# leonzheng2/Safe-Exploration-with-Simulator-in-RL-algorithms

Hardware: AMD Instinct MI355X
Metric: env-steps/sec (higher is better)
Workload: dtype f64; 1 GPU; ARS V2 iteration, 3-segment swimmer, 512 directions/GPU x 2 rollouts x H=1000 (BASELINE configs[2] per GPU); directions_total=512, directions_per_gpu=512, horizon=1000, segments=3, trajectory_capture=True, full_covariance=True, parallelism=directions sharded over 1 GPU(s), 1 all-gather/iteration, ranks_seen=1

## Files before the change

include/swimmer_hip.h:

```cpp
#ifndef SWIMMER_HIP_H
#define SWIMMER_HIP_H

#include <stdint.h>

#ifdef __cplusplus
extern "C" {
#endif

#define SW_ABI_VERSION 3
#define SW_MAX_SEGMENTS 8

#define SW_OK 0
#define SW_ERR_NULL 1
#define SW_ERR_SEGMENTS 2
#define SW_ERR_SIZE 3
#define SW_ERR_PARAM 4
#define SW_ERR_LAUNCH 5

#define SW_STATUS_OK 0
#define SW_STATUS_SINGULAR 1
#define SW_STATUS_NONFINITE 2
#define SW_STATUS_RANGE 4

#define SW_FLAG_ROLLOUT_LANE 1
// ... 110 lines not shown
int sw_ars_iteration_rollouts_f64(sw_ars_pipeline *pl, int slot, const sw_params *p,
                                  int64_t n_dir_total, int64_t dir_begin, int64_t n_dir,
                                  int32_t H, const double *deltas_host ,
                                  double *deltas_dev, const double *policy, double nu,
                                  const double *mean, const double *inv_std, double *returns,
                                  double *traj, double *moments, double *cov_acc,
                                  int32_t *status, void *stream);

int sw_ars_iteration_update_f64(sw_ars_pipeline *pl, int slot, const sw_params *p,
                                int64_t n_dir, const double *gathered, int32_t world,
                                int64_t chunk, int64_t rows_chunk, const double *deltas_dev,
                                double *policy, double alpha, double b, int64_t top_b,
                                double *running, int64_t n_new_states, double *mean,
                                double *inv_std, double *sigma_out, void *stream);

#ifdef __cplusplus
}
#endif
#endif
```

safe-exploration-with-simulator-in-rl-algorithms_amd/_lib.py:

```python
import ctypes
import os

import numpy as np
import torch

from . import _build

ABI_VERSION = 3
MAX_SEGMENTS = 8

ERR_NAMES = {0: "SW_OK", 1: "SW_ERR_NULL", 2: "SW_ERR_SEGMENTS", 3: "SW_ERR_SIZE",
             4: "SW_ERR_PARAM", 5: "SW_ERR_LAUNCH"}
STATUS_SINGULAR = 1
STATUS_NONFINITE = 2
STATUS_RANGE = 4
FLAG_ROLLOUT_LANE = 1
FLAG_ROLLOUT_QUAD = 2
FLAG_MODEL_TWIN = 4
COST_ABS_OBS = 0
COST_MAX_ABS_THETADOT = 1


class SwParams(ctypes.Structure):
    _fields_ = [("n", ctypes.c_int32), ("flags", ctypes.c_int32), ("l_i", ctypes.c_double),
# ... 88 lines not shown
                                                     ctypes.c_void_p, ctypes.c_int64,
                                                     ctypes.c_int64, ctypes.c_int64,
                                                     ctypes.c_int32, ctypes.c_void_p,
                                                     ctypes.c_void_p, ctypes.c_void_p,
                                                     ctypes.c_double] + [ctypes.c_void_p] * 8),
    "sw_ars_iteration_update_f64": (ctypes.c_int, [ctypes.c_void_p, ctypes.c_int,
                                                   ctypes.c_void_p, ctypes.c_int64,
                                                   ctypes.c_void_p, ctypes.c_int32,
                                                   ctypes.c_int64, ctypes.c_int64,
                                                   ctypes.c_void_p, ctypes.c_void_p,
                                                   ctypes.c_double, ctypes.c_double,
                                                   ctypes.c_int64, ctypes.c_void_p,
                                                   ctypes.c_int64, ctypes.c_void_p,
                                                   ctypes.c_void_p, ctypes.c_void_p,
                                                   ctypes.c_void_p]),
    "sw_ars_update_gathered_f64": (ctypes.c_int, [ctypes.c_void_p, ctypes.c_int64,
                                                  ctypes.c_void_p, ctypes.c_int32,
                                                  ctypes.c_int64, ctypes.c_int64,
                                                  ctypes.c_void_p, ctypes.c_void_p,
                                                  ctypes.c_double, ctypes.c_double,
                                                  ctypes.c_int64, ctypes.c_void_p,
                                                  ctypes.c_int64, ctypes.c_void_p,
                                                  ctypes.c_void_p, ctypes.c_void_p,
                                                  ctypes.c_void_p]),
}
EXPORTED_SYMBOLS = tuple(_PROTOTYPES)


def library_path():
    return _build.LIB_PATH
# ... 73 lines not shown
```

safe-exploration-with-simulator-in-rl-algorithms_amd/ars/ars_agent.py:

```python
import os

import numpy as np
import torch
import torch.distributed as dist

from .. import kernels
from .._lib import (SwParams, SwimmerHipError, kernel_flags, numpy_global_uniform_pm1,
                    require_gpu)
from .database import Database
from .environment import Environment
from . import sharding as _sh
from .sharding import (all_gather_segments, returns_from_segments, segment_len,
                       shard_bounds)


class ARSAgent(object):

    def __init__(self, real_env_param, agent_param, data_path=None, seed=None,
                 guess_param=None, approx_error=None, sim_thresh=None, *, device=None,
                 process_group=None, record_trajectories=False, full_covariance=True,
                 top_b=0, rollout_kernel="auto", direct_rccl=None):
        if agent_param.safe:
            raise NotImplementedError(
                "safe exploration (ars_agent.py:144-157) gates every real rollout on a "
# ... 177 lines not shown
                           self.agent_param.b, 0, sigma_out=self._sigma)

    def run_iteration_async(self, deltas=None, want_returns=True):
        ap = self.agent_param
        i = self._pipe.next_slot()
        self._it += 1
        self._pipe.host_slot_wait(i)
        if self.record_trajectories:
            self._policy_snapshot = self._policy.cpu().numpy()
        host = self._deltas_host_np[i]
        if deltas is None:
            numpy_global_uniform_pm1(host)
        else:
            host[...] = deltas
        self._deltas, self._traj = self._deltas2[i], self._traj2[i]
        self._pipe.rollouts(i, self.params, ap.N, self.lo, self.n_local, ap.H,
                            self._deltas_host[i], self._deltas, self._policy, ap.nu,
                            self._mean, self._inv_std, self._returns_local, self._traj,
                            self._moments_local,
                            self._cov_acc if self._traj is not None else None, self._status)
        if self._coll_events is not None and (self.world > 1 or _sh._FORCE_COLLECTIVE):
            e0 = torch.cuda.Event(enable_timing=True)
            e1 = torch.cuda.Event(enable_timing=True)
            e0.record()
            gathered = self._exchange()
            e1.record()
            self._coll_events.append((e0, e1))
        else:
            gathered = self._exchange()
        n_new = 2 * ap.N * ap.H
        self._pipe.update(i, self.params, ap.N, gathered, self.world, self.chunk,
                          self.rows_chunk, self._deltas, self._policy, ap.alpha, ap.b,
                          self.top_b, self._running, n_new, self._mean, self._inv_std,
                          self._sigma)
        if self.v2:
            self.n_saved_states += n_new
        if self.record_trajectories and self._traj is not None:
            self.database.add_device_batch(self._traj.clone(),
                                           self._rollout_policies(host.copy()))
        if not want_returns:
            return None
        return returns_from_segments(gathered, ap.N, self.world, self.chunk)

    def _rollout_policies(self, deltas):
        P = self._policy_snapshot
        out = np.empty((2 * self.n_local, self.m, self.d))
        nd = self.agent_param.nu * np.asarray(deltas)[self.lo:self.hi]
        out[0::2] = P + nd
        out[1::2] = P - nd
# ... 95 lines not shown
```

safe-exploration-with-simulator-in-rl-algorithms_amd/csrc/swimmer_kernels.hip:

```cpp
#include <hip/hip_runtime.h>
#include <math.h>
#include <stdint.h>
#include <climits>
#include <cstdlib>
#include <cstring>
#include <new>
#include <type_traits>
#include <utility>
#include <vector>

#include <chrono>
#include "../../include/swimmer_hip.h"
#include "swimmer_device.h"
#include "swimmer_quad3.h"
#include "swimmer_oct3.h"
#include "swimmer_row.h"
#include "swimmer_twin.h"

#define SW_PIN_LOOP(PAD) asm volatile(".p2align 6\n\t.fill %0, 4, 0xbf800000" ::"n"(PAD))
#ifndef SW_OCT_UNROLL
#define SW_OCT_UNROLL 8
#endif
#ifdef SW_OCT_LOOP_PAD
constexpr int oct_loop_pad(bool, bool) { return SW_OCT_LOOP_PAD; }
// ... 1840 lines not shown
}

constexpr int kTopBMaxDirs = 6144;

__device__ __forceinline__ bool rank_used_global(const GatherView &g, int32_t n_dir, int64_t top_b, int32_t i)
{
    const double ki = fmax(ret_at(g, i, 0), ret_at(g, i, 1));
    int64_t rank = 0;
    for (int32_t j = 0; j < n_dir; ++j) {
        const double kj = fmax(ret_at(g, j, 0), ret_at(g, j, 1));
        rank += (kj > ki) || (kj == ki && j > i);
    }
    return rank < top_b;
}

constexpr int kUpdMaxDirs = kTopBMaxDirs;
constexpr int kTopBSortDirs = 2048;

template <int BLOCK>
__global__ void __launch_bounds__(BLOCK)
ars_update_kernel(int d, int md, int32_t n_dir, GatherView gv,
                  const double *__restrict__ deltas, double *__restrict__ policy, double alpha,
                  double b, int64_t top_b, double *__restrict__ running, double n_new,
                  double *__restrict__ mean, double *__restrict__ inv_std,
                  double *__restrict__ sigma_out)
{
    __shared__ double sh2[BLOCK / kWave][2];
    __shared__ double rp_s[kUpdMaxDirs], rm_s[kUpdMaxDirs];
    __shared__ unsigned char flag[kUpdMaxDirs];
    const int e = blockIdx.x;
// ... 4 lines not shown
        double dcol[kMaxPer];
        if (in_lds) {
#pragma unroll
            for (int q = 0; q < kMaxPer; ++q) {
                const int32_t i = threadIdx.x + q * BLOCK;
                dcol[q] = (i < n_dir) ? deltas[(int64_t)i * md + e] : 0.0;
            }
            for (int32_t i = threadIdx.x; i < n_dir; i += BLOCK) {
                rp_s[i] = ret_at(gv, i, 0);
                rm_s[i] = ret_at(gv, i, 1);
            }
            __syncthreads();
            if (select && n_dir <= kTopBSortDirs) {
                __shared__ double skey[kTopBSortDirs];
                __shared__ uint16_t sidx[kTopBSortDirs];
                uint32_t P2 = 2;
                while (P2 < (uint32_t)n_dir) P2 <<= 1;
                for (uint32_t i = threadIdx.x; i < P2; i += BLOCK) {
                    double k = -HUGE_VAL;
                    if (i < (uint32_t)n_dir) {
                        const double a = rp_s[i], b = rm_s[i];
                        k = (b > a) ? b : a;
                        k = (k != k) ? HUGE_VAL : k;
                    }
                    skey[i] = k;
                    sidx[i] = (uint16_t)i;
                }
                __syncthreads();
                for (uint32_t k = 2; k <= P2; k <<= 1) {
                    for (uint32_t j = k >> 1; j > 0; j >>= 1) {
                        for (uint32_t t = threadIdx.x; t < P2 / 2; t += BLOCK) {
                            const uint32_t lo = ((t & ~(j - 1u)) << 1) | (t & (j - 1u)), hi = lo | j;
                            const double ka = skey[lo], kb = skey[hi];
                            const uint32_t ia = sidx[lo], ib = sidx[hi];
                            const bool a_first = (ia < (uint32_t)n_dir) &&
                                                 ((ib >= (uint32_t)n_dir) || ka > kb || (ka == kb && ia > ib));
                            const bool best_first = (lo & k) == 0;
                            if (a_first != best_first) {
                                skey[lo] = kb;
                                skey[hi] = ka;
                                sidx[lo] = (uint16_t)ib;
                                sidx[hi] = (uint16_t)ia;
                            }
                        }
                        __syncthreads();
                    }
                }
                for (uint32_t pos = threadIdx.x; pos < P2; pos += BLOCK) {
                    const uint32_t i = sidx[pos];
                    if (i < (uint32_t)n_dir) flag[i] = (int64_t)pos < top_b;
                }
                __syncthreads();
            } else if (select) {
                for (int32_t i = threadIdx.x; i < n_dir; i += BLOCK) {
                    const double ki = fmax(rp_s[i], rm_s[i]);
                    int32_t rank = 0;
                    for (int32_t j = 0; j < n_dir; ++j) {
                        const double kj = fmax(rp_s[j], rm_s[j]);
                        rank += (kj > ki) || (kj == ki && j > i);
                    }
                    flag[i] = rank < top_b;
                }
                __syncthreads();
            }
        }
        auto rplus = [&](int32_t i) { return in_lds ? rp_s[i] : ret_at(gv, i, 0); };
        auto rminus = [&](int32_t i) { return in_lds ? rm_s[i] : ret_at(gv, i, 1); };
// ... 2 lines not shown
            return in_lds ? (flag[i] != 0) : rank_used_global(gv, n_dir, top_b, i);
        };
        double s = 0.0, cnt = 0.0;
        for (int32_t i = threadIdx.x; i < n_dir; i += BLOCK)
            if (dir_used(i)) {
                s += rplus(i) + rminus(i);
                cnt += 2.0;
            }
        block_sum2<BLOCK>(s, cnt, sh2);
        const double mu = s / cnt;
        double v = 0.0, g = 0.0;
        if (in_lds) {
#pragma unroll
            for (int q = 0; q < kMaxPer; ++q) {
                const int32_t i = threadIdx.x + q * BLOCK;
                if (i < n_dir && dir_used(i)) {
                    const double rp = rp_s[i], rm = rm_s[i];
                    const double a = rp - mu, c = rm - mu;
                    v += a * a + c * c;
                    g = __builtin_fma(rp - rm, dcol[q], g);
                }
            }
        } else {
            for (int32_t i = threadIdx.x; i < n_dir; i += BLOCK)
                if (dir_used(i)) {
                    const double rp = rplus(i), rm = rminus(i);
                    const double a = rp - mu, c = rm - mu;
                    v += a * a + c * c;
                    g = __builtin_fma(rp - rm, deltas[(int64_t)i * md + e], g);
                }
        }
        block_sum2<BLOCK>(v, g, sh2);
        if (threadIdx.x == 0) {
            const double sigma = sqrt(v / cnt);
            const double div = (top_b > 0) ? 0.5 * cnt : b;
            const double grad = g / (div * sigma);
            policy[e] = policy[e] + alpha * grad;
            if (e == 0 && sigma_out) *sigma_out = sigma;
        }
    } else if (running != nullptr) {
        constexpr int kMaxCols = 2 * (2 * SW_MAX_SEGMENTS + 2);
        constexpr int kMaxGroups = BLOCK / 12;
        __shared__ double part[kMaxGroups][kMaxCols];
        __shared__ double bsum[kMaxCols];
        const int cols = 2 * d, G = BLOCK / cols;
        const int rg = threadIdx.x / cols, j = threadIdx.x - rg * cols;
        const int32_t total = gv.world * gv.rows_chunk;
        if (rg < G) {
            double acc = 0.0;
            for (int32_t g0 = rg; g0 < total; g0 += 8 * G) {
                double v[8];
#pragma unroll
                for (int q = 0; q < 8; ++q) {
                    const int32_t g = g0 + q * G;
// ... 4 lines not shown
                    }
                }
#pragma unroll
                for (int q = 0; q < 8; ++q) acc += v[q];
            }
            part[rg][j] = acc;
        }
        __syncthreads();
        if (threadIdx.x < cols) {
            double t = part[0][threadIdx.x];
            for (int g = 1; g < G; ++g) t += part[g][threadIdx.x];
            bsum[threadIdx.x] = t;
        }
        __syncthreads();
        const double n0 = running[0], n1 = n0 + n_new;
        if (threadIdx.x < d && n_new > 0.0) {
            const int c_ = threadIdx.x;
            const double s1 = bsum[c_], s2 = bsum[d + c_];
            const double mb = s1 / n_new;
            const double m2b = __builtin_fma(-s1, mb, s2);
            const double mr = running[1 + c_], m2 = running[1 + d + c_];
            const double delta = mb - mr;
            const double mr1 = __builtin_fma(delta, n_new / n1, mr);
            const double m21 = (m2 + m2b) + delta * delta * (n0 * (n_new / n1));
            running[1 + c_] = mr1;
            running[1 + d + c_] = m21;
            const double c = (c_ >= 2 && (c_ & 1) == 0) ? kHalfPi : 0.0;
            mean[c_] = c + mr1;
            inv_std[c_] = 1.0 / sqrt(m21 / (n1 - 1.0));
        }
        __syncthreads();
        if (threadIdx.x == 0) running[0] = n1;
    }
}

__global__ void __launch_bounds__(256) issue_probe_kernel(int32_t trips, int32_t mode, double *out)
{
    double a0 = 1.0 + threadIdx.x, a1 = a0 + 1, a2 = a0 + 2, a3 = a0 + 3, a4 = a0 + 4, a5 = a0 + 5,
           a6 = a0 + 6, a7 = a0 + 7;
    const double m = 1.0000001, c = 1e-9;
    int b0 = threadIdx.x, b1 = b0 + 1, b2 = b0 + 2, b3 = b0 + 3, b4 = b0 + 4, b5 = b0 + 5, b6 = b0 + 6,
        b7 = b0 + 7;
#define SW_FMA8 "v_fma_f64 %0, %0, %8, %9\n v_fma_f64 %1, %1, %8, %9\n v_fma_f64 %2, %2, %8, %9\n" \
                "v_fma_f64 %3, %3, %8, %9\n v_fma_f64 %4, %4, %8, %9\n v_fma_f64 %5, %5, %8, %9\n" \
                "v_fma_f64 %6, %6, %8, %9\n v_fma_f64 %7, %7, %8, %9\n"
#define SW_MOV8 "v_mov_b32 %0, %1\n v_mov_b32 %1, %2\n v_mov_b32 %2, %3\n v_mov_b32 %3, %4\n" \
                "v_mov_b32 %4, %5\n v_mov_b32 %5, %6\n v_mov_b32 %6, %7\n v_mov_b32 %7, %0\n"
    if (mode == 0) {
        for (int32_t t = 0; t < trips; ++t)
// ... 374 lines not shown
        case 6: SW_LAUNCH_SAFE_ROW(6); break;
        case 7: SW_LAUNCH_SAFE_ROW(7); break;
        default: SW_LAUNCH_SAFE_ROW(8); break;
        }
#undef SW_LAUNCH_SAFE_ROW
        return launch_status();
    }
    const unsigned grid = (unsigned)((n_roll + kRollBlock - 1) / kRollBlock);
    SW_DISPATCH_N(real->n, hipLaunchKernelGGL((safe_rollout_kernel<NN>), dim3(grid), dim3(kRollBlock), 0,
                                              (hipStream_t)stream, Cr, Cs, n_roll, H, policies, cost_kind,
                                              cost_index, sim_thresh, real_thresh, returns, traj, first_refused,
                                              violations, status));
    return launch_status();
}

static int launch_ars_rollouts(const sw_params *p, int64_t dir_begin, int64_t n_dir, int32_t H,
                               const double *policy, const double *deltas, double nu,
                               const double *mean, const double *inv_std, double *returns,
                               double *traj, double *moments, int32_t *status, void *stream,
                               const SideJob *side, bool *side_taken)
{
    int rc = validate_params(p);
    if (rc) return rc;
    if (n_dir < 0 || H < 0 || dir_begin < 0) return SW_ERR_SIZE;
    if (side_taken) *side_taken = false;
    if (n_dir == 0) return SW_OK;
    if (!policy || !deltas || !returns) return SW_ERR_NULL;
    if ((mean == nullptr) != (inv_std == nullptr)) return SW_ERR_NULL;
    const sw::Consts C = make_consts(p);
    const int64_t n_roll = 2 * n_dir;
    if (use_oct3(p, n_roll, H, traj != nullptr)) {
        unsigned grid = (unsigned)((n_roll + kMomGroup - 1) / kMomGroup);
        SideJob sj = side ? *side : kNoSide;
        grid += side_attach_cov(sj, grid, kOctBlock, 2 * p->n + 2);
        if (side_taken) *side_taken = side != nullptr;
        SW_DISPATCH_OCT(true, traj != nullptr, moments != nullptr,
                        (hipStream_t)stream, C, n_roll, H, policy, deltas, dir_begin, nu, mean,
                        inv_std, (const double *)nullptr, returns, traj, (double *)nullptr,
                        moments, status, sj);
        return launch_status();
    }
    if (use_quad3(p, n_roll, H, traj != nullptr)) {
        unsigned grid = (unsigned)((n_roll + kMomGroup - 1) / kMomGroup);
        SideJob sj = side ? *side : kNoSide;
        grid += side_attach_cov(sj, grid, kRollBlock, 2 * p->n + 2);
        if (side_taken) *side_taken = side != nullptr;
        SW_DISPATCH_QUAD(true, traj != nullptr, moments != nullptr,
                         (hipStream_t)stream, C, n_roll, H, policy, deltas, dir_begin, nu, mean,
                         inv_std, (const double *)nullptr, returns, traj, (double *)nullptr,
                         moments, status, sj);
// ... 235 lines not shown
    hipEvent_t h2d_done[SW_PIPELINE_SLOTS] = {};
    bool h2d_valid[SW_PIPELINE_SLOTS] = {};
    uint32_t *flag_host = nullptr, *flag_dev = nullptr;
    uint32_t launches = 0;
    hipStream_t last_main = nullptr;
    bool main_seen = false;
    int timing = 0;
    int64_t timing_launches = 0;
    std::vector<std::pair<hipEvent_t, hipEvent_t>> timed;
    const double *cov_traj = nullptr;
    double *cov_acc = nullptr;
    int64_t cov_rolls = 0;
    int32_t cov_H = 0;
    int cov_block = 0;
    sw_params cov_params = {};
};

namespace {

__global__ void flag_kernel(uint32_t *flag, uint32_t value)
{
    __hip_atomic_store(flag, value, __ATOMIC_RELAXED, __HIP_MEMORY_SCOPE_SYSTEM);
}

int wait_flag(const sw_ars_pipeline *pl, uint32_t need)
{
    const volatile uint32_t *f = pl->flag_host;
    auto last = std::chrono::steady_clock::now();
    for (int64_t spins = 0;; ++spins) {
        if ((int32_t)(*f - need) >= 0) return SW_OK;
// ... 26 lines not shown
    if (!out) return SW_ERR_NULL;
    sw_ars_pipeline *pl = new (std::nothrow) sw_ars_pipeline();
    if (!pl) return SW_ERR_LAUNCH;
    const unsigned evf = hipEventDisableTiming;
    int prio_least = 0, prio_greatest = 0;
    (void)hipDeviceGetStreamPriorityRange(&prio_least, &prio_greatest);
    bool ok = hipStreamCreateWithPriority(&pl->copy, hipStreamNonBlocking, prio_greatest) == hipSuccess &&
              hipHostMalloc((void **)&pl->flag_host, 64, hipHostMallocMapped | hipHostMallocCoherent) ==
                  hipSuccess;
    if (ok) {
        *pl->flag_host = 0u;
        ok = hipHostGetDevicePointer((void **)&pl->flag_dev, pl->flag_host, 0) == hipSuccess;
    }
    for (int i = 0; i < SW_PIPELINE_SLOTS && ok; ++i)
        ok = hipEventCreateWithFlags(&pl->h2d_done[i], evf) == hipSuccess;
    if (!ok) {
        sw_ars_pipeline_destroy(pl);
        return SW_ERR_LAUNCH;
    }
    *out = pl;
    return SW_OK;
}

void sw_ars_pipeline_destroy(sw_ars_pipeline *pl)
{
    if (!pl) return;
    if (pl->copy) (void)hipStreamSynchronize(pl->copy);
    if (pl->main_seen) (void)hipStreamSynchronize(pl->last_main);
    for (auto &e : pl->timed) {
        (void)hipEventDestroy(e.first);
        (void)hipEventDestroy(e.second);
    }
    for (int i = 0; i < SW_PIPELINE_SLOTS; ++i)
        if (pl->h2d_done[i]) (void)hipEventDestroy(pl->h2d_done[i]);
    if (pl->copy) (void)hipStreamDestroy(pl->copy);
    if (pl->flag_host) (void)hipHostFree(pl->flag_host);
    delete pl;
}

int sw_ars_pipeline_slots(void) { return SW_PIPELINE_SLOTS; }

int sw_ars_pipeline_host_slot_wait(sw_ars_pipeline *pl, int slot)
{
    if (!pl) return SW_ERR_NULL;
    if (slot < 0 || slot >= SW_PIPELINE_SLOTS) return SW_ERR_SIZE;
    if (pl->h2d_valid[slot] && hipEventSynchronize(pl->h2d_done[slot]) != hipSuccess)
        return SW_ERR_LAUNCH;
    return SW_OK;
}

int sw_ars_pipeline_sync_cov(sw_ars_pipeline *pl)
// ... 28 lines not shown
        if (hipEventSynchronize(e.second) != hipSuccess) return SW_ERR_LAUNCH;
        float ms = 0.f;
        if (hipEventElapsedTime(&ms, e.first, e.second) != hipSuccess) return SW_ERR_LAUNCH;
        tot += ms;
    }
    *launches = (int64_t)pl->timed.size();
    *mean_ms = pl->timed.empty() ? 0.0 : tot / (double)pl->timed.size();
    return SW_OK;
}

int sw_ars_pipeline_next_slot(sw_ars_pipeline *pl)
{
    return pl ? (int)(pl->launches % (uint32_t)SW_PIPELINE_SLOTS) : -1;
}

int sw_ars_iteration_rollouts_f64(sw_ars_pipeline *pl, int slot, const sw_params *p,
                                  int64_t n_dir_total, int64_t dir_begin, int64_t n_dir, int32_t H,
                                  const double *deltas_host, double *deltas_dev,
                                  const double *policy, double nu, const double *mean,
                                  const double *inv_std, double *returns, double *traj,
                                  double *moments, double *cov_acc, int32_t *status, void *stream)
{
    int rc = check_params(p);
    if (rc) return rc;
    if (!pl || !deltas_host || !deltas_dev) return SW_ERR_NULL;
    if (n_dir < 0 || dir_begin < 0 || H < 0 || n_dir_total < dir_begin + n_dir) return SW_ERR_SIZE;
    const uint32_t k = pl->launches;
    if (slot != (int)(k % (uint32_t)SW_PIPELINE_SLOTS)) return SW_ERR_SIZE;
    if (cov_acc && !traj && n_dir > 0) return SW_ERR_NULL;
    hipStream_t main = (hipStream_t)stream;
    if (pl->main_seen && pl->last_main != main) {
        if (hipStreamSynchronize(pl->last_main) != hipSuccess) return SW_ERR_LAUNCH;
    }
    pl->last_main = main;
    pl->main_seen = true;
    const size_t bytes = (size_t)n_dir_total * (size_t)((p->n - 1) * (2 * p->n + 2)) * sizeof(double);
// ... 35 lines not shown
    }
    if (ride) {
        sj.cov_traj = pl->cov_traj;
        sj.cov_acc = pl->cov_acc;
        sj.cov_rolls = pl->cov_rolls;
        sj.cov_H = pl->cov_H;
    }
    bool taken = false;
    if (!quad && !row) {
        hipLaunchKernelGGL(flag_kernel, dim3(1), dim3(1), 0, main, pl->flag_dev, k);
        rc = launch_status();
        if (rc) return rc;
        sj = kNoSide;
    }
    rc = launch_ars_rollouts(p, dir_begin, n_dir, H, policy, deltas_dev, nu, mean, inv_std,
                             returns, traj, moments, status, stream, &sj, &taken);
    if (timed_launch) {
        (void)hipEventRecord(ev.second, main);
        pl->timed.push_back(ev);
    }
    if (rc) return rc;
    if (ride) pl->cov_traj = nullptr;
    pl->launches = k + 1u;
    if (cov_acc) {
        pl->cov_traj = traj;
        pl->cov_acc = cov_acc;
        pl->cov_rolls = 2 * n_dir;
        pl->cov_H = H;
        pl->cov_block = block;
        pl->cov_params = *p;
    }
    return SW_OK;
}

int sw_ars_iteration_update_f64(sw_ars_pipeline *pl, int slot, const sw_params *p, int64_t n_dir,
                                const double *gathered, int32_t world, int64_t chunk,
                                int64_t rows_chunk, const double *deltas_dev, double *policy,
                                double alpha, double b, int64_t top_b, double *running,
                                int64_t n_new_states, double *mean, double *inv_std,
                                double *sigma_out, void *stream)
{
    if (!pl) return SW_ERR_NULL;
    if (slot < 0 || slot >= SW_PIPELINE_SLOTS) return SW_ERR_SIZE;
    return sw_ars_update_gathered_f64(p, n_dir, gathered, world, chunk, rows_chunk, deltas_dev,
                                      policy, alpha, b, top_b, running, n_new_states, mean,
                                      inv_std, sigma_out, stream);
}

}
// ... 1 lines not shown
```

safe-exploration-with-simulator-in-rl-algorithms_amd/kernels.py:

```python
import ctypes

import torch

from . import _lib
from ._lib import SwParams, check, load, ptr, require_gpu, stream_ptr


def _f64(shape, device):
    return torch.empty(shape, dtype=torch.float64, device=device)


def _want(t, name, shape):
    if t.dtype != torch.float64 or tuple(t.shape) != tuple(shape):
        raise _lib.SwimmerHipError(f"{name}: expected float64 tensor of shape {tuple(shape)}, "
                                   f"got {t.dtype} {tuple(t.shape)}")
    return t


def reset(p: SwParams, n_env: int, device="cuda:0", out=None):
    require_gpu()
    state = _f64((p.d, n_env), device) if out is None else _want(out, "out", (p.d, n_env))
    check(load().sw_reset_f64(ctypes.byref(p), n_env, ptr(state), stream_ptr()), "sw_reset_f64")
    return state

# ... 371 lines not shown
        ms, n = ctypes.c_double(), ctypes.c_int64()
        check(load().sw_ars_pipeline_rollout_ms(self._h, ctypes.byref(ms), ctypes.byref(n)),
              "sw_ars_pipeline_rollout_ms")
        return ms.value, n.value

    def rollouts(self, slot, p, n_dir_total, dir_begin, n_dir, H, deltas_host, deltas_dev, policy,
                 nu, mean, inv_std, returns, traj, moments, cov_acc, status):
        if not deltas_host.is_pinned() or not deltas_host.is_contiguous():
            raise _lib.SwimmerHipError("deltas_host must be a contiguous pinned CPU tensor")
        check(load().sw_ars_iteration_rollouts_f64(
            self._h, slot, ctypes.byref(p), n_dir_total, dir_begin, n_dir, H,
            ctypes.c_void_p(deltas_host.data_ptr()), ptr(deltas_dev), ptr(policy), float(nu),
            ptr(mean), ptr(inv_std), ptr(returns), ptr(traj), ptr(moments), ptr(cov_acc),
            ptr(status), stream_ptr()), "sw_ars_iteration_rollouts_f64")

    def update(self, slot, p, n_dir, gathered, world, chunk, rows_chunk, deltas_dev, policy,
               alpha, b, top_b, running, n_new_states, mean, inv_std, sigma_out):
        check(load().sw_ars_iteration_update_f64(
            self._h, slot, ctypes.byref(p), n_dir, ptr(gathered), int(world), int(chunk),
            int(rows_chunk), ptr(deltas_dev), ptr(policy), float(alpha), float(b), int(top_b),
            ptr(running), int(n_new_states), ptr(mean), ptr(inv_std), ptr(sigma_out),
            stream_ptr()), "sw_ars_iteration_update_f64")
```

Before: 4.534 billion env-steps/s.

## Add single-call ARS iteration with optional fused rollout-plus-update kernel

```diff
diff --git a/include/swimmer_hip.h b/include/swimmer_hip.h
--- a/include/swimmer_hip.h
+++ b/include/swimmer_hip.h
@@ -148,6 +148,13 @@
                                 double *running, int64_t n_new_states, double *mean,
                                 double *inv_std, double *sigma_out, void *stream);
 
+int sw_ars_iteration_f64(sw_ars_pipeline *pl, int slot, const sw_params *p, int64_t n_dir, int32_t H,
+                         const double *deltas_host , double *deltas_dev, double *policy,
+                         double nu, double *mean, double *inv_std, double *returns, double *traj,
+                         double *moments, double *cov_acc, int32_t *status, double alpha, double b,
+                         int64_t top_b, double *running, int64_t n_new_states, double *sigma_out,
+                         void *stream);
+
 #ifdef __cplusplus
 }
 #endif
diff --git a/safe-exploration-with-simulator-in-rl-algorithms_amd/_lib.py b/safe-exploration-with-simulator-in-rl-algorithms_amd/_lib.py
--- a/safe-exploration-with-simulator-in-rl-algorithms_amd/_lib.py
+++ b/safe-exploration-with-simulator-in-rl-algorithms_amd/_lib.py
@@ -126,6 +126,11 @@
                                                    ctypes.c_int64, ctypes.c_void_p,
                                                    ctypes.c_void_p, ctypes.c_void_p,
                                                    ctypes.c_void_p]),
+    "sw_ars_iteration_f64": (ctypes.c_int, [ctypes.c_void_p, ctypes.c_int, ctypes.c_void_p, ctypes.c_int64,
+                                            ctypes.c_int32] + [ctypes.c_void_p] * 3 + [ctypes.c_double]
+                             + [ctypes.c_void_p] * 7 + [ctypes.c_double, ctypes.c_double, ctypes.c_int64,
+                                                        ctypes.c_void_p, ctypes.c_int64, ctypes.c_void_p,
+                                                        ctypes.c_void_p]),
     "sw_ars_update_gathered_f64": (ctypes.c_int, [ctypes.c_void_p, ctypes.c_int64,
                                                   ctypes.c_void_p, ctypes.c_int32,
                                                   ctypes.c_int64, ctypes.c_int64,
diff --git a/safe-exploration-with-simulator-in-rl-algorithms_amd/ars/ars_agent.py b/safe-exploration-with-simulator-in-rl-algorithms_amd/ars/ars_agent.py
--- a/safe-exploration-with-simulator-in-rl-algorithms_amd/ars/ars_agent.py
+++ b/safe-exploration-with-simulator-in-rl-algorithms_amd/ars/ars_agent.py
@@ -215,6 +215,14 @@
         else:
             host[...] = deltas
         self._deltas, self._traj = self._deltas2[i], self._traj2[i]
+        n_new = 2 * ap.N * ap.H
+        if self.world == 1 and not _sh._FORCE_COLLECTIVE:
+            self._pipe.iteration(i, self.params, ap.N, ap.H, self._deltas_host[i], self._deltas, self._policy,
+                                 ap.nu, self._mean, self._inv_std, self._returns_local, self._traj,
+                                 self._moments_local, self._cov_acc if self._traj is not None else None,
+                                 self._status, ap.alpha, ap.b, self.top_b, self._running, n_new,
+                                 self._sigma)
+            return self._finish_iteration(host, n_new, self._send, want_returns)
         self._pipe.rollouts(i, self.params, ap.N, self.lo, self.n_local, ap.H,
                             self._deltas_host[i], self._deltas, self._policy, ap.nu,
                             self._mean, self._inv_std, self._returns_local, self._traj,
@@ -229,11 +237,14 @@
             self._coll_events.append((e0, e1))
         else:
             gathered = self._exchange()
-        n_new = 2 * ap.N * ap.H
         self._pipe.update(i, self.params, ap.N, gathered, self.world, self.chunk,
                           self.rows_chunk, self._deltas, self._policy, ap.alpha, ap.b,
                           self.top_b, self._running, n_new, self._mean, self._inv_std,
                           self._sigma)
+        return self._finish_iteration(host, n_new, gathered, want_returns)
+
+    def _finish_iteration(self, host, n_new, gathered, want_returns):
+        ap = self.agent_param
         if self.v2:
             self.n_saved_states += n_new
         if self.record_trajectories and self._traj is not None:
diff --git a/safe-exploration-with-simulator-in-rl-algorithms_amd/csrc/swimmer_kernels.hip b/safe-exploration-with-simulator-in-rl-algorithms_amd/csrc/swimmer_kernels.hip
--- a/safe-exploration-with-simulator-in-rl-algorithms_amd/csrc/swimmer_kernels.hip
+++ b/safe-exploration-with-simulator-in-rl-algorithms_amd/csrc/swimmer_kernels.hip
@@ -1878,6 +1878,82 @@
     return rank < top_b;
 }
 
+template <int NT>
+__device__ __forceinline__ void topb_flags_bitonic(const double *rp_s, const double *rm_s, int32_t n_dir,
+                                                   int64_t top_b, double *skey, uint16_t *sidx, unsigned char *flag)
+{
+    uint32_t P2 = 2;
+    while (P2 < (uint32_t)n_dir) P2 <<= 1;
+    for (uint32_t i = threadIdx.x; i < P2; i += NT) {
+        double k = -HUGE_VAL;
+        if (i < (uint32_t)n_dir) {
+            const double a = rp_s[i], b = rm_s[i];
+            k = (b > a) ? b : a;
+            k = (k != k) ? HUGE_VAL : k;
+        }
+        skey[i] = k;
+        sidx[i] = (uint16_t)i;
+    }
+    __syncthreads();
+    for (uint32_t k = 2; k <= P2; k <<= 1) {
+        for (uint32_t j = k >> 1; j > 0; j >>= 1) {
+            for (uint32_t t = threadIdx.x; t < P2 / 2; t += NT) {
+                const uint32_t lo = ((t & ~(j - 1u)) << 1) | (t & (j - 1u)), hi = lo | j;
+                const double ka = skey[lo], kb = skey[hi];
+                const uint32_t ia = sidx[lo], ib = sidx[hi];
+                const bool a_first = (ia < (uint32_t)n_dir) &&
+                                     ((ib >= (uint32_t)n_dir) || ka > kb || (ka == kb && ia > ib));
+                const bool best_first = (lo & k) == 0;
+                if (a_first != best_first) {
+                    skey[lo] = kb;
+                    skey[hi] = ka;
+                    sidx[lo] = (uint16_t)ib;
+                    sidx[hi] = (uint16_t)ia;
+                }
+            }
+            __syncthreads();
+        }
+    }
+    for (uint32_t pos = threadIdx.x; pos < P2; pos += NT) {
+        const uint32_t i = sidx[pos];
+        if (i < (uint32_t)n_dir) flag[i] = (int64_t)pos < top_b;
+    }
+    __syncthreads();
+}
+
+__device__ __forceinline__ void upd_spread_terms(double rp, double rm, double mu, double dv, double &v, double &g)
+{
+    const double a = rp - mu, c = rm - mu;
+    v += a * a + c * c;
+    g = __builtin_fma(rp - rm, dv, g);
+}
+
+__device__ __forceinline__ void upd_policy_entry(int e, double v, double g, double cnt, int64_t top_b, double b,
+                                                 double alpha, double *policy, double *sigma_out)
+{
+    const double sigma = sqrt(v / cnt);
+    const double div = (top_b > 0) ? 0.5 * cnt : b;
+    const double grad = g / (div * sigma);
+    policy[e] = policy[e] + alpha * grad;
+    if (e == 0 && sigma_out) *sigma_out = sigma;
+}
+
+__device__ __forceinline__ void upd_stats_merge(int c_, int d, double s1, double s2, double n0, double n1,
+                                                double n_new, double *running, double *mean, double *inv_std)
+{
+    const double mb = s1 / n_new;
+    const double m2b = __builtin_fma(-s1, mb, s2);
+    const double mr = running[1 + c_], m2 = running[1 + d + c_];
+    const double delta = mb - mr;
+    const double mr1 = __builtin_fma(delta, n_new / n1, mr);
+    const double m21 = (m2 + m2b) + delta * delta * (n0 * (n_new / n1));
+    running[1 + c_] = mr1;
+    running[1 + d + c_] = m21;
+    const double c = (c_ >= 2 && (c_ & 1) == 0) ? kHalfPi : 0.0;
+    mean[c_] = c + mr1;
+    inv_std[c_] = 1.0 / sqrt(m21 / (n1 - 1.0));
+}
+
 constexpr int kUpdMaxDirs = kTopBMaxDirs;
 constexpr int kTopBSortDirs = 2048;
 
@@ -1912,43 +1988,7 @@
             if (select && n_dir <= kTopBSortDirs) {
                 __shared__ double skey[kTopBSortDirs];
                 __shared__ uint16_t sidx[kTopBSortDirs];
-                uint32_t P2 = 2;
-                while (P2 < (uint32_t)n_dir) P2 <<= 1;
-                for (uint32_t i = threadIdx.x; i < P2; i += BLOCK) {
-                    double k = -HUGE_VAL;
-                    if (i < (uint32_t)n_dir) {
-                        const double a = rp_s[i], b = rm_s[i];
-                        k = (b > a) ? b : a;
-                        k = (k != k) ? HUGE_VAL : k;
-                    }
-                    skey[i] = k;
-                    sidx[i] = (uint16_t)i;
-                }
-                __syncthreads();
-                for (uint32_t k = 2; k <= P2; k <<= 1) {
-                    for (uint32_t j = k >> 1; j > 0; j >>= 1) {
-                        for (uint32_t t = threadIdx.x; t < P2 / 2; t += BLOCK) {
-                            const uint32_t lo = ((t & ~(j - 1u)) << 1) | (t & (j - 1u)), hi = lo | j;
-                            const double ka = skey[lo], kb = skey[hi];
-                            const uint32_t ia = sidx[lo], ib = sidx[hi];
-                            const bool a_first = (ia < (uint32_t)n_dir) &&
-                                                 ((ib >= (uint32_t)n_dir) || ka > kb || (ka == kb && ia > ib));
-                            const bool best_first = (lo & k) == 0;
-                            if (a_first != best_first) {
-                                skey[lo] = kb;
-                                skey[hi] = ka;
-                                sidx[lo] = (uint16_t)ib;
-                                sidx[hi] = (uint16_t)ia;
-                            }
-                        }
-                        __syncthreads();
-                    }
-                }
-                for (uint32_t pos = threadIdx.x; pos < P2; pos += BLOCK) {
-                    const uint32_t i = sidx[pos];
-                    if (i < (uint32_t)n_dir) flag[i] = (int64_t)pos < top_b;
-                }
-                __syncthreads();
+                topb_flags_bitonic<BLOCK>(rp_s, rm_s, n_dir, top_b, skey, sidx, flag);
             } else if (select) {
                 for (int32_t i = threadIdx.x; i < n_dir; i += BLOCK) {
                     const double ki = fmax(rp_s[i], rm_s[i]);
@@ -1981,30 +2021,14 @@
 #pragma unroll
             for (int q = 0; q < kMaxPer; ++q) {
                 const int32_t i = threadIdx.x + q * BLOCK;
-                if (i < n_dir && dir_used(i)) {
-                    const double rp = rp_s[i], rm = rm_s[i];
-                    const double a = rp - mu, c = rm - mu;
-                    v += a * a + c * c;
-                    g = __builtin_fma(rp - rm, dcol[q], g);
-                }
+                if (i < n_dir && dir_used(i)) upd_spread_terms(rp_s[i], rm_s[i], mu, dcol[q], v, g);
             }
         } else {
             for (int32_t i = threadIdx.x; i < n_dir; i += BLOCK)
-                if (dir_used(i)) {
-                    const double rp = rplus(i), rm = rminus(i);
-                    const double a = rp - mu, c = rm - mu;
-                    v += a * a + c * c;
-                    g = __builtin_fma(rp - rm, deltas[(int64_t)i * md + e], g);
-                }
+                if (dir_used(i)) upd_spread_terms(rplus(i), rminus(i), mu, deltas[(int64_t)i * md + e], v, g);
         }
         block_sum2<BLOCK>(v, g, sh2);
-        if (threadIdx.x == 0) {
-            const double sigma = sqrt(v / cnt);
-            const double div = (top_b > 0) ? 0.5 * cnt : b;
-            const double grad = g / (div * sigma);
-            policy[e] = policy[e] + alpha * grad;
-            if (e == 0 && sigma_out) *sigma_out = sigma;
-        }
+        if (threadIdx.x == 0) upd_policy_entry(e, v, g, cnt, top_b, b, alpha, policy, sigma_out);
     } else if (running != nullptr) {
         constexpr int kMaxCols = 2 * (2 * SW_MAX_SEGMENTS + 2);
         constexpr int kMaxGroups = BLOCK / 12;
@@ -2039,25 +2063,356 @@
         }
         __syncthreads();
         const double n0 = running[0], n1 = n0 + n_new;
-        if (threadIdx.x < d && n_new > 0.0) {
-            const int c_ = threadIdx.x;
-            const double s1 = bsum[c_], s2 = bsum[d + c_];
-            const double mb = s1 / n_new;
-            const double m2b = __builtin_fma(-s1, mb, s2);
-            const double mr = running[1 + c_], m2 = running[1 + d + c_];
-            const double delta = mb - mr;
-            const double mr1 = __builtin_fma(delta, n_new / n1, mr);
-            const double m21 = (m2 + m2b) + delta * delta * (n0 * (n_new / n1));
-            running[1 + c_] = mr1;
-            running[1 + d + c_] = m21;
-            const double c = (c_ >= 2 && (c_ & 1) == 0) ? kHalfPi : 0.0;
-            mean[c_] = c + mr1;
-            inv_std[c_] = 1.0 / sqrt(m21 / (n1 - 1.0));
-        }
+        if (threadIdx.x < d && n_new > 0.0)
+            upd_stats_merge(threadIdx.x, d, bsum[threadIdx.x], bsum[d + threadIdx.x], n0, n1, n_new, running, mean,
+                            inv_std);
         __syncthreads();
         if (threadIdx.x == 0) running[0] = n1;
     }
 }
+
+#ifndef SW_OCT3F_LOOP_PAD
+#define SW_OCT3F_LOOP_PAD 6
+#endif
+constexpr int32_t kFusedMaxDirs = kTopBSortDirs;
+
+struct FusedUpdate {
+    const double *deltas;
+    double *policy;
+    double *mean, *inv_std, *running, *sigma_out;
+    uint32_t *retired;
+    double alpha, b, n_new;
+    int64_t top_b;
+    int32_t n_dir;
+};
+
+template <int VB>
+__device__ __forceinline__ void fused_update_tail(const FusedUpdate &U, const double *returns, const double *mom,
+                                                  int32_t rows)
+{
+    constexpr int NT = kOctBlock, D = 8, MD = 16, NWV = VB / kWave;
+    constexpr int NP = NWV / (NT / 32);
+    static_assert(NWV % (NT / 32) == 0, "virtual waves per 32-lane half");
+    __shared__ double rp_s[kFusedMaxDirs], rm_s[kFusedMaxDirs];
+    __shared__ unsigned char flag[kFusedMaxDirs];
+    __shared__ double skey[kFusedMaxDirs];
+    __shared__ uint16_t sidx[kFusedMaxDirs];
+    __shared__ double wsum[2 + MD][NWV];
+    constexpr int COLS = 2 * D, G = VB / COLS;
+    __shared__ double part[G][COLS];
+    __shared__ double bsum[COLS];
+    const int tid = threadIdx.x, half = tid / 32, l = tid % 32;
+    const int32_t n_dir = U.n_dir;
+    const bool select = U.top_b > 0 && U.top_b < n_dir;
+
+    for (int32_t i = tid; i < n_dir; i += NT) {
+        rp_s[i] = returns[2 * i];
+        rm_s[i] = returns[2 * i + 1];
+    }
+    double sacc[VB / NT];
+#pragma unroll
+    for (int k = 0; k < VB / NT; ++k) {
+        const int vt = tid + k * NT, rg = vt / COLS, j = vt - rg * COLS;
+        double acc = 0.0;
+        for (int32_t g0 = rg; g0 < rows; g0 += 8 * G) {
+            double v[8];
+#pragma unroll
+            for (int q = 0; q < 8; ++q) {
+                const int32_t g = g0 + q * G;
+                v[q] = (g < rows) ? mom[(int64_t)g * COLS + j] : 0.0;
+            }
+#pragma unroll
+            for (int q = 0; q < 8; ++q) acc += v[q];
+        }
+        sacc[k] = acc;
+    }
+#pragma unroll
+    for (int k = 0; k < VB / NT; ++k) {
+        const int vt = tid + k * NT, rg = vt / COLS;
+        part[rg][vt - rg * COLS] = sacc[k];
+    }
+    __syncthreads();
+    if (select) topb_flags_bitonic<NT>(rp_s, rm_s, n_dir, U.top_b, skey, sidx, flag);
+    auto used = [&](int32_t i) { return !select || flag[i] != 0; };
+    auto wave_total = [&](double x) {
+#pragma unroll
+        for (int off = 16; off > 0; off >>= 1) x += __shfl_down(x, off, 32);
+        return x;
+    };
+#pragma unroll
+    for (int p = 0; p < NP; ++p) {
+        const int w = half + 4 * p;
+        double s[2] = {0.0, 0.0}, cnt[2] = {0.0, 0.0};
+#pragma unroll
+        for (int h = 0; h < 2; ++h)
+            for (int32_t i = w * kWave + l + 32 * h; i < n_dir; i += VB)
+                if (used(i)) {
+                    s[h] += rp_s[i] + rm_s[i];
+                    cnt[h] += 2.0;
+                }
+        const double st = wave_total(s[0] + s[1]), ct = wave_total(cnt[0] + cnt[1]);
+        if (l == 0) {
+            wsum[0][w] = st;
+            wsum[1][w] = ct;
+        }
+    }
+    __syncthreads();
+    double s = 0.0, cnt = 0.0;
+    for (int w = 0; w < NWV; ++w) {
+        s += wsum[0][w];
+        cnt += wsum[1][w];
+    }
+    const double mu = s / cnt;
+    __syncthreads();
+#pragma unroll
+    for (int p = 0; p < NP; ++p) {
+        const int w = half + 4 * p;
+        double v[2] = {0.0, 0.0}, g[2][MD];
+#pragma unroll
+        for (int h = 0; h < 2; ++h)
+#pragma unroll
+            for (int e = 0; e < MD; ++e) g[h][e] = 0.0;
+        for (int32_t i0 = w * kWave + l; i0 < n_dir; i0 += 2 * VB) {
+            double dv[2][2][MD];
+#pragma unroll
+            for (int st = 0; st < 2; ++st)
+#pragma unroll
+                for (int h = 0; h < 2; ++h) {
+                    const int32_t i = i0 + st * VB + 32 * h;
+#pragma unroll
+                    for (int e = 0; e < MD; ++e) dv[st][h][e] = (i < n_dir) ? U.deltas[(int64_t)i * MD + e] : 0.0;
+                }
+#pragma unroll
+            for (int st = 0; st < 2; ++st)
+#pragma unroll
+                for (int h = 0; h < 2; ++h) {
+                    const int32_t i = i0 + st * VB + 32 * h;
+                    if (i < n_dir && used(i)) {
+#pragma unroll
+                        for (int e = 0; e < MD; ++e) {
+                            double ve = v[h];
+                            upd_spread_terms(rp_s[i], rm_s[i], mu, dv[st][h][e], ve, g[h][e]);
+                            if (e == 0) v[h] = ve;
+                        }
+                    }
+                }
+        }
+        const double vt = wave_total(v[0] + v[1]);
+        if (l == 0) wsum[0][w] = vt;
+#pragma unroll
+        for (int e = 0; e < MD; ++e) {
+            const double gt = wave_total(g[0][e] + g[1][e]);
+            if (l == 0) wsum[2 + e][w] = gt;
+        }
+    }
+    __syncthreads();
+    if (tid < MD) {
+        double v = 0.0, g = 0.0;
+        for (int w = 0; w < NWV; ++w) {
+            v += wsum[0][w];
+            g += wsum[2 + tid][w];
+        }
+        upd_policy_entry(tid, v, g, cnt, U.top_b, U.b, U.alpha, U.policy, U.sigma_out);
+    }
+    if (U.running != nullptr) {
+        if (tid < COLS) {
+            double t = part[0][tid];
+            for (int g = 1; g < G; ++g) t += part[g][tid];
+            bsum[tid] = t;
+        }
+        __syncthreads();
+        const double n0 = U.running[0], n1 = n0 + U.n_new;
+        if (tid < D && U.n_new > 0.0)
+            upd_stats_merge(tid, D, bsum[tid], bsum[D + tid], n0, n1, U.n_new, U.running, U.mean, U.inv_std);
+        __syncthreads();
+        if (tid == 0) U.running[0] = n1;
+    }
+}
+
+template <int VB>
+__global__ void __launch_bounds__(kOctBlock)
+rollout_oct3f_kernel(sw::Consts C, int64_t n_roll, int32_t H, const double *policy,
+                     const double *__restrict__ deltas, double nu, const double *mean, const double *inv_std,
+                     double *returns, double *__restrict__ traj, double *moments, int32_t *__restrict__ status,
+                     SideJob side, FusedUpdate U)
+{
+    side_flag(side);
+    if (blockIdx.x >= side.first_cov_block) {
+        side_cov_tile<8, kOctBlock>(side);
+        return;
+    }
+    __builtin_amdgcn_s_setprio(3);
+    constexpr int D = 8, M = 2;
+    const int tid = threadIdx.x, lane = tid & (kWave - 1), wave = tid / kWave;
+    const int q = lane & 3;
+    const int seg = (q == 3) ? 0 : q;
+    const bool cosine = (lane & 8) != 0;
+    const int64_t r_raw = (int64_t)blockIdx.x * kMomGroup + wave * 8 + (lane >> 4) * 2 + ((lane >> 2) & 1);
+    const bool valid = r_raw < n_roll;
+    const int64_t r = valid ? r_raw : n_roll - 1;
+    const sw::OctLane O = sw::oct3_lane(C, seg, cosine);
+    const int cth = 2 + 2 * seg, cthd = 3 + 2 * seg;
+
+    const int seg1 = (seg + 1) % 3, seg2 = (seg + 2) % 3;
+    const int cols[D] = {0, 1, cth, cthd, 2 + 2 * seg1, 3 + 2 * seg1, 2 + 2 * seg2, 3 + 2 * seg2};
+    double V[D], nbias;
+    load_policy_row<D, M, true>(policy, deltas + (r >> 1) * (M * D), (r & 1) ? -1.0 : 1.0, nu, mean, inv_std,
+                                C.c12, seg, cols, V, nbias);
+    const double VPu = cosine ? V[1] : V[0], VPv = cosine ? V[0] : V[1];
+
+    double th = kHalfPi, thd = 0.0, Pu = 0.0, Pv = 0.0;
+
+    const uint32_t kDrop = 0xfffffff0u;
+    const bool rec = !cosine && q < 3;
+    const uint32_t off_th = rec ? (uint32_t)(((int64_t)cth * n_roll + r) * 8) : kDrop;
+    const uint32_t off_thd = rec ? (uint32_t)(((int64_t)cthd * n_roll + r) * 8) : kDrop;
+    const uint32_t off_g = (q == 0) ? (uint32_t)(((int64_t)(cosine ? 1 : 0) * n_roll + r) * 8) : kDrop;
+    const uint32_t slab = (uint32_t)(D * n_roll * 8);
+    const __amdgpu_buffer_rsrc_t trs = __builtin_amdgcn_make_buffer_rsrc(
+        traj, 0, (int)(uint32_t)((int64_t)H * slab), 0x00020000);
+    uint32_t soff = 0;
+    auto store_cell = [&](double v, uint32_t voff) {
+        typedef int v2i __attribute__((ext_vector_type(2)));
+        union { double d; v2i i; } u;
+        u.d = v;
+        __builtin_amdgcn_raw_buffer_store_b64(u.i, trs, (int)voff, (int)soff, SW_TRAJ_STORE_AUX);
+    };
+
+    const int designation = cosine ? 1 : 0;
+    double thmax = 0.0, det = 1.0;
+    sw::OctTrig A;
+    A.r = th;
+    A.kd = 0.0;
+    sw::oct3_renorm(A, designation, thmax);
+    double m1th = 0.0, m2th = 0.0, m1thd = 0.0, m2thd = 0.0, m1g = 0.0, m2g = 0.0;
+    double w1 = sw::dpp_f64<sw::kDppNext1>(thd), w2 = sw::dpp_f64<sw::kDppNext2>(thd);
+    double Th = __builtin_fma(V[2], th, nbias);
+    Th = __builtin_fma(V[4], sw::dpp_f64<sw::kDppNext1>(th), Th);
+    Th = __builtin_fma(V[6], sw::dpp_f64<sw::kDppNext2>(th), Th);
+    const double hV2 = C.h * V[2], hV4 = C.h * V[4], hV6 = C.h * V[6];
+    sw::OctGeo G = sw::oct3_geometry(A), Gn;
+    double magic = 6755399441055744.0;
+    asm volatile("" : "+v"(magic));
+    auto one_step = [&](const sw::OctGeo &Gc, sw::OctGeo &Gx) {
+        A.r = __builtin_fma(C.h, thd, A.r);
+        const unsigned long long outside = sw::oct3_range_test(A.r);
+        double tq = __builtin_fma(VPu, Pu, Th);
+        tq = __builtin_fma(VPv, Pv, tq);
+        tq = __builtin_fma(V[3], thd, tq);
+        tq = __builtin_fma(V[5], w1, tq);
+        tq = __builtin_fma(V[7], w2, tq);
+        Th = __builtin_fma(hV2, thd, Th);
+        Th = __builtin_fma(hV4, w1, Th);
+        Th = __builtin_fma(hV6, w2, Th);
+        sw::oct3_keep_reduced(A, thmax, magic, designation, outside);
+        const double th_next = __builtin_fma(A.kd, sw::kPio2Hi, A.r);
+        Gx = sw::oct3_geometry(A);
+        det = sw::oct3_dynamics(C, O, Gc, Pu, Pv, thd, w1, w2, tq);
+        th = th_next;
+        m1g += Pu;
+        store_cell(th, off_th);
+        store_cell(thd, off_thd);
+        store_cell(Pu, off_g);
+        soff += slab;
+        const double a = th - kHalfPi;
+        m1th += a;
+        m2th = __builtin_fma(a, a, m2th);
+        m1thd += thd;
+        m2thd = __builtin_fma(thd, thd, m2thd);
+        m2g = __builtin_fma(Pu, Pu, m2g);
+        w1 = sw::dpp_f64<sw::kDppNext1>(thd);
+        w2 = sw::dpp_f64<sw::kDppNext2>(thd);
+        Pv = sw::dpp_row_f64<sw::kDppRowRor8>(Pu);
+    };
+    int32_t t = 0;
+    SW_PIN_LOOP(SW_OCT3F_LOOP_PAD);
+#if SW_OCT_UNROLL == 8
+    for (; t + 8 <= H; t += 8) {
+        one_step(G, Gn);
+        one_step(Gn, G);
+        one_step(G, Gn);
+        one_step(Gn, G);
+        one_step(G, Gn);
+        one_step(Gn, G);
+        one_step(G, Gn);
+        one_step(Gn, G);
+    }
+#endif
+    for (; t + 4 <= H; t += 4) {
+        one_step(G, Gn);
+        one_step(Gn, G);
+        one_step(G, Gn);
+        one_step(Gn, G);
+    }
+    for (; t + 2 <= H; t += 2) {
+        one_step(G, Gn);
+        one_step(Gn, G);
+    }
+    if (t < H) one_step(G, Gn);
+    thmax = fmax(thmax, fabs(th));
+
+    int code = ((det > 0.0) ? 0 : SW_STATUS_SINGULAR) |
+               ((isfinite(th) && isfinite(thd) && isfinite(Pu) && isfinite(Pv)) ? 0 : SW_STATUS_NONFINITE) |
+               ((thmax < sw::kAngleLimit) ? 0 : SW_STATUS_RANGE);
+    code |= __builtin_amdgcn_mov_dpp(code, sw::kDppNext1, 0xf, 0xf, true) |
+            __builtin_amdgcn_mov_dpp(code, sw::kDppNext2, 0xf, 0xf, true);
+    code |= __builtin_amdgcn_mov_dpp(code, sw::kDppRowRor8, 0xf, 0xf, true);
+    const double sg_other = sw::dpp_row_f64<sw::kDppRowRor8>(m1g);
+    if (valid && !cosine && q == 0) {
+        const double total = __builtin_fma(C.dirx, m1g, C.diry * sg_other);
+        __hip_atomic_store(returns + r, (code & SW_STATUS_RANGE) ? __builtin_nan("") : total, __ATOMIC_RELAXED,
+                           __HIP_MEMORY_SCOPE_AGENT);
+        if (status) status[r] = code;
+    }
+    {
+        __shared__ double shm[kOctBlock / kWave][16][6];
+        if (!valid) m1th = m2th = m1thd = m2thd = m1g = m2g = 0.0;
+#pragma unroll
+        for (int k = 0; k < 3; ++k) {
+            const int off = (k == 0) ? 4 : (k == 1 ? 16 : 32);
+            m1th += __shfl_xor(m1th, off, kWave);
+            m2th += __shfl_xor(m2th, off, kWave);
+            m1thd += __shfl_xor(m1thd, off, kWave);
+            m2thd += __shfl_xor(m2thd, off, kWave);
+            m1g += __shfl_xor(m1g, off, kWave);
+            m2g += __shfl_xor(m2g, off, kWave);
+        }
+        if (lane < 16) {
+            shm[wave][lane][0] = m1th;
+            shm[wave][lane][1] = m2th;
+            shm[wave][lane][2] = m1thd;
+            shm[wave][lane][3] = m2thd;
+            shm[wave][lane][4] = m1g;
+            shm[wave][lane][5] = m2g;
+        }
+        __syncthreads();
+        if (tid < 3) {
+            double *row = moments + (int64_t)blockIdx.x * (2 * D);
+            auto put = [&](int j, double v) { __hip_atomic_store(row + j, v, __ATOMIC_RELAXED, __HIP_MEMORY_SCOPE_AGENT); };
+            put(2 + 2 * tid, shm[0][tid][0] + shm[1][tid][0]);
+            put(D + 2 + 2 * tid, shm[0][tid][1] + shm[1][tid][1]);
+            put(3 + 2 * tid, shm[0][tid][2] + shm[1][tid][2]);
+            put(D + 3 + 2 * tid, shm[0][tid][3] + shm[1][tid][3]);
+            if (tid < 2) {
+                const int src = tid * 8;
+                put(tid, shm[0][src][4] + shm[1][src][4]);
+                put(D + tid, shm[0][src][5] + shm[1][src][5]);
+            }
+        }
+    }
+    asm volatile("s_waitcnt vmcnt(0)" ::: "memory");
+    __builtin_amdgcn_fence(__ATOMIC_RELEASE, "workgroup");
+    __syncthreads();
+    __shared__ uint32_t retired;
+    const uint32_t n_blocks = (uint32_t)((n_roll + kMomGroup - 1) / kMomGroup);
+    if (tid == 0) retired = atomicAdd(U.retired, 1u);
+    __syncthreads();
+    if (retired != n_blocks - 1u) return;
+    __threadfence();
+    fused_update_tail<VB>(U, returns, moments, (int32_t)n_blocks);
+    if (tid == 0) *U.retired = 0u;
+}
+
 
 __global__ void __launch_bounds__(256) issue_probe_kernel(int32_t trips, int32_t mode, double *out)
 {
@@ -2462,16 +2817,24 @@
     return launch_status();
 }
 
+static bool fused_update_fits(const sw_params *p, int64_t n_dir, int32_t H, const double *traj,
+                              const double *moments, int64_t dir_begin)
+{
+    return dir_begin == 0 && n_dir > 0 && n_dir <= kFusedMaxDirs && traj && moments &&
+           use_oct3(p, 2 * n_dir, H, true);
+}
+
 static int launch_ars_rollouts(const sw_params *p, int64_t dir_begin, int64_t n_dir, int32_t H,
                                const double *policy, const double *deltas, double nu,
                                const double *mean, const double *inv_std, double *returns,
                                double *traj, double *moments, int32_t *status, void *stream,
-                               const SideJob *side, bool *side_taken)
+                               const SideJob *side, bool *side_taken, const FusedUpdate *fused = nullptr)
 {
     int rc = validate_params(p);
     if (rc) return rc;
     if (n_dir < 0 || H < 0 || dir_begin < 0) return SW_ERR_SIZE;
     if (side_taken) *side_taken = false;
+    if (fused && !fused_update_fits(p, n_dir, H, traj, moments, dir_begin)) return SW_ERR_SIZE;
     if (n_dir == 0) return SW_OK;
     if (!policy || !deltas || !returns) return SW_ERR_NULL;
     if ((mean == nullptr) != (inv_std == nullptr)) return SW_ERR_NULL;
@@ -2482,6 +2845,17 @@
         SideJob sj = side ? *side : kNoSide;
         grid += side_attach_cov(sj, grid, kOctBlock, 2 * p->n + 2);
         if (side_taken) *side_taken = side != nullptr;
+        if (fused) {
+            if (n_dir >= kUpdWideFrom)
+                hipLaunchKernelGGL(rollout_oct3f_kernel<kUpdBlockWide>, dim3(grid), dim3(kOctBlock), 0,
+                                   (hipStream_t)stream, C, n_roll, H, policy, deltas, nu, mean, inv_std, returns,
+                                   traj, moments, status, sj, *fused);
+            else
+                hipLaunchKernelGGL(rollout_oct3f_kernel<kUpdBlock>, dim3(grid), dim3(kOctBlock), 0,
+                                   (hipStream_t)stream, C, n_roll, H, policy, deltas, nu, mean, inv_std, returns,
+                                   traj, moments, status, sj, *fused);
+            return launch_status();
+        }
         SW_DISPATCH_OCT(true, traj != nullptr, moments != nullptr,
                         (hipStream_t)stream, C, n_roll, H, policy, deltas, dir_begin, nu, mean,
                         inv_std, (const double *)nullptr, returns, traj, (double *)nullptr,
@@ -2747,6 +3121,8 @@
     int32_t cov_H = 0;
     int cov_block = 0;
     sw_params cov_params = {};
+    bool fuse_update = false;
+    uint32_t *retired = nullptr;
 };
 
 namespace {
@@ -2803,6 +3179,10 @@
     }
     for (int i = 0; i < SW_PIPELINE_SLOTS && ok; ++i)
         ok = hipEventCreateWithFlags(&pl->h2d_done[i], evf) == hipSuccess;
+    const char *fuse_env = getenv("SWIMMER_FUSED_UPDATE");
+    pl->fuse_update = fuse_env && fuse_env[0] == '1';
+    ok = ok && hipMalloc((void **)&pl->retired, sizeof(uint32_t)) == hipSuccess &&
+         hipMemset(pl->retired, 0, sizeof(uint32_t)) == hipSuccess;
     if (!ok) {
         sw_ars_pipeline_destroy(pl);
         return SW_ERR_LAUNCH;
@@ -2824,6 +3204,7 @@
         if (pl->h2d_done[i]) (void)hipEventDestroy(pl->h2d_done[i]);
     if (pl->copy) (void)hipStreamDestroy(pl->copy);
     if (pl->flag_host) (void)hipHostFree(pl->flag_host);
+    if (pl->retired) (void)hipFree(pl->retired);
     delete pl;
 }
 
@@ -2882,12 +3263,11 @@
     return pl ? (int)(pl->launches % (uint32_t)SW_PIPELINE_SLOTS) : -1;
 }
 
-int sw_ars_iteration_rollouts_f64(sw_ars_pipeline *pl, int slot, const sw_params *p,
-                                  int64_t n_dir_total, int64_t dir_begin, int64_t n_dir, int32_t H,
-                                  const double *deltas_host, double *deltas_dev,
-                                  const double *policy, double nu, const double *mean,
-                                  const double *inv_std, double *returns, double *traj,
-                                  double *moments, double *cov_acc, int32_t *status, void *stream)
+static int iteration_rollouts(sw_ars_pipeline *pl, int slot, const sw_params *p, int64_t n_dir_total,
+                              int64_t dir_begin, int64_t n_dir, int32_t H, const double *deltas_host,
+                              double *deltas_dev, const double *policy, double nu, const double *mean,
+                              const double *inv_std, double *returns, double *traj, double *moments,
+                              double *cov_acc, int32_t *status, void *stream, const FusedUpdate *fused)
 {
     int rc = check_params(p);
     if (rc) return rc;
@@ -2953,7 +3333,7 @@
         sj = kNoSide;
     }
     rc = launch_ars_rollouts(p, dir_begin, n_dir, H, policy, deltas_dev, nu, mean, inv_std,
-                             returns, traj, moments, status, stream, &sj, &taken);
+                             returns, traj, moments, status, stream, &sj, &taken, fused);
     if (timed_launch) {
         (void)hipEventRecord(ev.second, main);
         pl->timed.push_back(ev);
@@ -2972,6 +3352,44 @@
     return SW_OK;
 }
 
+int sw_ars_iteration_rollouts_f64(sw_ars_pipeline *pl, int slot, const sw_params *p,
+                                  int64_t n_dir_total, int64_t dir_begin, int64_t n_dir, int32_t H,
+                                  const double *deltas_host, double *deltas_dev,
+                                  const double *policy, double nu, const double *mean,
+                                  const double *inv_std, double *returns, double *traj,
+                                  double *moments, double *cov_acc, int32_t *status, void *stream)
+{
+    return iteration_rollouts(pl, slot, p, n_dir_total, dir_begin, n_dir, H, deltas_host, deltas_dev, policy, nu,
+                              mean, inv_std, returns, traj, moments, cov_acc, status, stream, nullptr);
+}
+
+int sw_ars_iteration_f64(sw_ars_pipeline *pl, int slot, const sw_params *p, int64_t n_dir, int32_t H,
+                         const double *deltas_host, double *deltas_dev, double *policy, double nu,
+                         double *mean, double *inv_std, double *returns, double *traj, double *moments,
+                         double *cov_acc, int32_t *status, double alpha, double b, int64_t top_b,
+                         double *running, int64_t n_new_states, double *sigma_out, void *stream)
+{
+    if (!pl) return SW_ERR_NULL;
+    int rc = check_params(p);
+    if (rc) return rc;
+    if (n_dir <= 0 || n_dir > INT32_MAX / 4 || n_new_states < 0) return SW_ERR_SIZE;
+    if (!policy || !deltas_dev || !returns) return SW_ERR_NULL;
+    if (running && (!moments || !mean || !inv_std)) return SW_ERR_NULL;
+    const int64_t rows = moments ? (2 * n_dir + kMomGroup - 1) / kMomGroup : 0;
+    if (pl->fuse_update && running && fused_update_fits(p, n_dir, H, traj, moments, 0)) {
+        const FusedUpdate fu{deltas_dev, policy, mean, inv_std, running, sigma_out, pl->retired,
+                             alpha, b, (double)n_new_states, top_b, (int32_t)n_dir};
+        return iteration_rollouts(pl, slot, p, n_dir, 0, n_dir, H, deltas_host, deltas_dev, policy, nu, mean,
+                                  inv_std, returns, traj, moments, cov_acc, status, stream, &fu);
+    }
+    rc = iteration_rollouts(pl, slot, p, n_dir, 0, n_dir, H, deltas_host, deltas_dev, policy, nu, mean, inv_std,
+                            returns, traj, moments, cov_acc, status, stream, nullptr);
+    if (rc) return rc;
+    const GatherView gv{returns, moments, 0, (int32_t)n_dir, (int32_t)rows, 1};
+    return launch_update(p, n_dir, gv, deltas_dev, policy, alpha, b, top_b, running, n_new_states, mean, inv_std,
+                         sigma_out, stream);
+}
+
 int sw_ars_iteration_update_f64(sw_ars_pipeline *pl, int slot, const sw_params *p, int64_t n_dir,
                                 const double *gathered, int32_t world, int64_t chunk,
                                 int64_t rows_chunk, const double *deltas_dev, double *policy,
diff --git a/safe-exploration-with-simulator-in-rl-algorithms_amd/kernels.py b/safe-exploration-with-simulator-in-rl-algorithms_amd/kernels.py
--- a/safe-exploration-with-simulator-in-rl-algorithms_amd/kernels.py
+++ b/safe-exploration-with-simulator-in-rl-algorithms_amd/kernels.py
@@ -409,6 +409,16 @@
             ptr(mean), ptr(inv_std), ptr(returns), ptr(traj), ptr(moments), ptr(cov_acc),
             ptr(status), stream_ptr()), "sw_ars_iteration_rollouts_f64")
 
+    def iteration(self, slot, p, n_dir, H, deltas_host, deltas_dev, policy, nu, mean, inv_std, returns, traj,
+                  moments, cov_acc, status, alpha, b, top_b, running, n_new_states, sigma_out):
+        if not deltas_host.is_pinned() or not deltas_host.is_contiguous():
+            raise _lib.SwimmerHipError("deltas_host must be a contiguous pinned CPU tensor")
+        check(load().sw_ars_iteration_f64(
+            self._h, slot, ctypes.byref(p), n_dir, H, ctypes.c_void_p(deltas_host.data_ptr()), ptr(deltas_dev),
+            ptr(policy), float(nu), ptr(mean), ptr(inv_std), ptr(returns), ptr(traj), ptr(moments), ptr(cov_acc),
+            ptr(status), float(alpha), float(b), int(top_b), ptr(running), int(n_new_states), ptr(sigma_out),
+            stream_ptr()), "sw_ars_iteration_f64")
+
     def update(self, slot, p, n_dir, gathered, world, chunk, rows_chunk, deltas_dev, policy,
                alpha, b, top_b, running, n_new_states, mean, inv_std, sigma_out):
         check(load().sw_ars_iteration_update_f64(
```

New measurement: 4.532 billion env-steps/s, median of 6. About the same (-0.0%).
